# triq-org/spectroplot-js

Measured on AMD Instinct MI355X. Metric: STFT frames/sec (N=1024 cf32) + IQ MSamples/s end-to-end to RGBA, higher is better.
Workload: dtype f64; 1 GPU; 16 MSample cf32, N=1024, Blackman-Harris, Viridis, gain 6, range 30, spectrogram layout, 16384 frames per GPU; format=CF32, n=1024, samples_per_gpu=16777216, frames_per_gpu=16384, window=blackmanHarris, cmap=viridis, generator=trinoise seed=0x5EED0001 step=7321 gshift=11 amp=0.5 namp=0.02

## Files before the change

### include/spectroplot_hip.h

```cpp
#ifndef SPECTROPLOT_HIP_H
#define SPECTROPLOT_HIP_H

#include <stddef.h>
#include <stdint.h>

#ifdef __cplusplus
extern "C" {
#endif

#define SP_VERSION 100
#define SP_CB_HIST_SIZE 1000
#define SP_MAX_LUT 4096
#define SP_MAX_N (1 << 20)

enum sp_status {
    SP_OK = 0,
    SP_ERR_INVALID_ARG = -1,
    SP_ERR_NOT_POW2 = -2,
    SP_ERR_BYTE_LENGTH = -3,
    SP_ERR_UNSUPPORTED = -4,
    SP_ERR_NO_DEVICE = -5,
    SP_ERR_HIP = -6,
    SP_ERR_NOMEM = -7
};
// ... 73 lines not shown
    int32_t n;
    int32_t channel_mode, waterfall;
    double gain, range;
} sp_named_request;
int sp_render_named(sp_context *ctx, const sp_named_request *req, const uint8_t *bytes, size_t nbytes, int32_t width, const sp_reply *reply);
int sp_render_named_ex(sp_context *ctx, const sp_named_request *req, int32_t detector, const uint8_t *bytes, size_t nbytes, int32_t width,
                       const sp_reply *reply);
int sp_named_resolve(const char *window, const char *cmap, const char **window_name, const char **cmap_key, int32_t *lut_len);
int sp_context_plan_creations(const sp_context *ctx, int64_t *count);

int sp_plan_create(sp_context *ctx, const sp_request *req, sp_plan **plan);
void sp_plan_destroy(sp_plan *plan);
int sp_plan_execute(sp_plan *plan, const void *d_bytes, size_t nbytes, int32_t width, const sp_reply *d_reply);
int sp_plan_execute_from_host(sp_plan *plan, const uint8_t *bytes, size_t nbytes, int32_t width, const sp_reply *d_reply);
int sp_merge_replies(sp_context *ctx, const void *d_records, int32_t count, int32_t lut_len, uint64_t *d_c_hist, uint64_t *d_cb_hist,
                     double *d_dbfs_minmax);
int sp_merge_replies_batch(sp_context *ctx, const void *d_gathered, int32_t ranks, int32_t renders, int32_t lut_len, void *d_merged);
int sp_place_strips(sp_context *ctx, uint8_t *d_image, const uint8_t *d_strips, int32_t count, int32_t n, int32_t width,
                    int32_t slice_width, int32_t waterfall);
typedef struct sp_group sp_group;
enum sp_group_gather { SP_GROUP_GATHER_DEVICE = 0, SP_GROUP_GATHER_HOST = 1 };
int sp_group_create(const int32_t *devices, int32_t count, sp_group **group);
void sp_group_destroy(sp_group *group);
int sp_group_size(const sp_group *group);
int sp_group_render(sp_group *group, const sp_request *req, const uint8_t *bytes, size_t nbytes, int32_t width, const sp_reply *reply);
int sp_group_render_ex(sp_group *group, const sp_request *req, const uint8_t *bytes, size_t nbytes, int32_t width, const sp_reply *reply,
                       int32_t gather);
const char *sp_group_transport(const sp_group *group);
const char *sp_group_transport_note(const sp_group *group);
int sp_group_last_timings(const sp_group *group, double *render_ms, double *gather_ms, double *download_ms);
int sp_group_rccl_info(const sp_group *group, char *text, size_t capacity);
int sp_group_root_bytes(const sp_group *group, size_t *image_bytes, size_t *staging_bytes);
const char *sp_group_last_error(const sp_group *group);

typedef struct sp_batch_item {
    const void *bytes;
    size_t nbytes;
    int32_t width;
    int32_t reserved;
    sp_reply reply;
} sp_batch_item;
int sp_plan_execute_batch(sp_plan *plan, const sp_batch_item *items, int32_t count);
int sp_render_batch(sp_context *ctx, const sp_request *req, const sp_batch_item *items, int32_t count);
int sp_debug_batch_plan(int32_t format, int32_t n, int32_t lut_len, int32_t cu_count, const size_t *nbytes, const int32_t *widths,
                        int32_t count, int64_t *out, size_t capacity, size_t *used);

int sp_plan_debug_launch(const sp_plan *plan, size_t nbytes, int32_t width, const void *rgba, int64_t *out, size_t capacity, size_t *used);
int sp_debug_frames_launch(int32_t n, int32_t lut_len, int64_t count, int32_t cu_count, int32_t gf_fixed, int64_t *out, size_t capacity,
                           size_t *used);

const char *sp_plan_kernel_name(const sp_plan *plan);
const char *sp_plan_kernel_name_for(const sp_plan *plan, size_t nbytes, int32_t width);
int sp_plan_force_kernel(sp_plan *plan, int32_t which);

int sp_plan_execute_traces(sp_plan *plan, const void *d_bytes, size_t nbytes, int32_t width, double *d_trace_min, double *d_trace_max);
int sp_render_traces(sp_context *ctx, const sp_request *req, const uint8_t *bytes, size_t nbytes, int32_t width, double *trace_min,
                     double *trace_max);
const char *sp_plan_traces_kernel_name_for(const sp_plan *plan, size_t nbytes, int32_t width);

int sp_plan_execute_power(sp_plan *plan, const void *d_bytes, size_t nbytes, int32_t width, double *d_power);
int sp_plan_power_to_db(sp_plan *plan, const double *d_power, size_t count, double *d_db);
int sp_render_power(sp_context *ctx, const sp_request *req, const uint8_t *bytes, size_t nbytes, int32_t width, int32_t db, double *power);
const char *sp_plan_power_kernel_name_for(const sp_plan *plan, size_t nbytes, int32_t width);

int sp_power_mean(sp_context *ctx, const double *d_power, int32_t n, int32_t width, double *d_mean);
int sp_plan_execute_mean(sp_plan *plan, const void *d_bytes, size_t nbytes, int32_t width, double *d_mean);
int sp_render_mean(sp_context *ctx, const sp_request *req, const uint8_t *bytes, size_t nbytes, int32_t width, int32_t db, double *mean);
int sp_context_set_mean_window(sp_context *ctx, size_t bytes);
int sp_debug_exact_sum(const double *values, size_t count, double *sum);
const char *sp_plan_mean_kernel_name_for(const sp_plan *plan, size_t nbytes, int32_t width);

#define SP_MAX_BANDS 64
int sp_band_rows(int32_t n, double f_lo, double f_hi, int32_t *y0, int32_t *y1);
int sp_power_bands(sp_context *ctx, const double *d_power, int32_t n, int32_t width, const int32_t *bands, int32_t count, double *d_band);
int sp_plan_execute_bandpower(sp_plan *plan, const void *d_bytes, size_t nbytes, int32_t width, const int32_t *bands, int32_t count,
                              double *d_band);
int sp_render_bandpower(sp_context *ctx, const sp_request *req, const uint8_t *bytes, size_t nbytes, int32_t width, const int32_t *bands,
                        int32_t count, int32_t db, double *band);
const char *sp_plan_bandpower_kernel_name_for(const sp_plan *plan, size_t nbytes, int32_t width);

int sp_power_tracks(sp_context *ctx, const double *d_power, int32_t n, int32_t width, const int32_t *bands, int32_t count,
                    int32_t *d_row, double *d_peak);
int sp_plan_execute_track(sp_plan *plan, const void *d_bytes, size_t nbytes, int32_t width, const int32_t *bands, int32_t count,
                          int32_t *d_row, double *d_peak);
int sp_render_track(sp_context *ctx, const sp_request *req, const uint8_t *bytes, size_t nbytes, int32_t width, const int32_t *bands,
                    int32_t count, int32_t db, int32_t *row, double *peak);
const char *sp_plan_track_kernel_name_for(const sp_plan *plan, size_t nbytes, int32_t width);
int sp_debug_band_peak(const double *values, int32_t n, int32_t y0, int32_t y1, int32_t *row, double *peak);

#define SP_OCCUPANCY_TILE_ROWS 4096
int sp_power_occupancy(sp_context *ctx, const double *d_power, int32_t n, int32_t width, const double *d_threshold, const int32_t *bands,
                       int32_t count, uint32_t *d_rows, uint32_t *d_frames);
int sp_plan_execute_occupancy(sp_plan *plan, const void *d_bytes, size_t nbytes, int32_t width, const double *d_threshold,
                              const int32_t *bands, int32_t count, uint32_t *d_rows, uint32_t *d_frames);
int sp_render_occupancy(sp_context *ctx, const sp_request *req, const uint8_t *bytes, size_t nbytes, int32_t width, const double *threshold,
                        const int32_t *bands, int32_t count, uint32_t *rows, uint32_t *frames);
const char *sp_plan_occupancy_kernel_name_for(const sp_plan *plan, size_t nbytes, int32_t width);
int sp_debug_occupancy(const double *values, const double *thresholds, int32_t n, int32_t y0, int32_t y1, uint32_t *count);

int sp_plan_execute_index(sp_plan *plan, const void *d_bytes, size_t nbytes, int32_t width, const sp_reply *d_reply, uint8_t *d_index);
int sp_render_index(sp_context *ctx, const sp_request *req, const uint8_t *bytes, size_t nbytes, int32_t width, const sp_reply *reply,
                    uint8_t *index);
int sp_index_to_rgba(sp_context *ctx, const uint8_t *d_index, size_t pixels, const uint8_t *lut_rgb, int32_t lut_len, uint8_t *d_rgba);
const char *sp_plan_index_kernel_name_for(const sp_plan *plan, size_t nbytes, int32_t width);
int sp_plan_debug_index_launch(const sp_plan *plan, size_t nbytes, int32_t width, const void *index, int64_t *out, size_t capacity,
                               size_t *used);
// ... 31 lines not shown
```

### spectroplot-js_amd/binding.py

```python
import ctypes as C
import math
import os
import weakref
import subprocess

import numpy as np

_HERE = os.path.dirname(os.path.abspath(__file__))

SP_CB_HIST_SIZE = 1000
FORMATS = ["CU4", "CS4", "CU8", "CS8", "CU12", "CS12", "CU16", "CS16", "CU32", "CS32", "CU64", "CS64", "CF32", "CF64"]

SP_ERR_NOT_POW2 = -2
SP_ERR_BYTE_LENGTH = -3
SP_ERR_UNSUPPORTED = -4
SP_ERR_NO_DEVICE = -5
SP_ERR_INVALID_ARG = -1

DETECTORS = {"sample": 0, "peak": 1}


def detector_id(detector):
    if detector not in DETECTORS:
        raise SpectroplotError(SP_ERR_INVALID_ARG, "detector must be 'sample' or 'peak', not %r" % (detector,))
# ... 36 lines not shown
def build_library(force=False):
    target = lib_path()
    if force:
        subprocess.check_call(["make", "-s", "-C", _HERE, "clean"])
    subprocess.check_call(["make", "-s", "-C", _HERE])
    return target


class Library:
    _instance = None

    def __init__(self, path=None):
        path = path or lib_path()
        if not os.path.exists(path):
            raise SpectroplotError(SP_ERR_NO_DEVICE, "HIP library %s is missing: run __graft_entry__.build() first" % path)
        L = self.L = C.CDLL(path)
        self.path = path
        vp, i32, sz, dbl = C.c_void_p, C.c_int32, C.c_size_t, C.c_double
        L.sp_version.restype = C.c_int
        L.sp_status_string.restype = C.c_char_p
        L.sp_status_string.argtypes = [C.c_int]
        L.sp_last_error.restype = C.c_char_p
        L.sp_last_error.argtypes = [vp]
        L.sp_format_parse.argtypes = [C.c_char_p, C.POINTER(i32), C.POINTER(i32)]
        L.sp_format_element_size.argtypes = [i32]
        L.sp_slice_bounds.argtypes = [sz, i32, i32, i32, C.POINTER(sz), C.POINTER(sz)]
        L.sp_window.argtypes = [C.c_char_p, i32, vp, C.POINTER(dbl)]
        L.sp_twiddles.argtypes = [i32, vp, vp]
        L.sp_js_log10.restype = dbl
        L.sp_js_log10.argtypes = [dbl]
        L.sp_cmap_count.restype = C.c_int
        L.sp_cmap_key.restype = C.c_char_p
        L.sp_cmap_key.argtypes = [i32]
        L.sp_cmap.argtypes = [C.c_char_p, vp, i32, C.POINTER(i32)]
        L.sp_cmap_generate.argtypes = [C.c_char_p, i32, vp]
        L.sp_plan_execute_from_host.argtypes = [vp, vp, sz, i32, C.POINTER(_Reply)]
        L.sp_device_count.argtypes = [C.POINTER(i32)]
        L.sp_context_create.argtypes = [i32, C.POINTER(vp)]
        L.sp_context_destroy.argtypes = [vp]
        L.sp_context_destroy.restype = None
        L.sp_context_set_stream.argtypes = [vp, vp]
        L.sp_context_synchronize.argtypes = [vp]
        L.sp_render.argtypes = [vp, C.POINTER(_Request), vp, sz, i32, C.POINTER(_Reply)]
        L.sp_render_named.argtypes = [vp, C.POINTER(_NamedRequest), vp, sz, i32, C.POINTER(_Reply)]
        L.sp_named_resolve.argtypes = [C.c_char_p, C.c_char_p, C.POINTER(C.c_char_p), C.POINTER(C.c_char_p), C.POINTER(i32)]
        L.sp_context_plan_creations.argtypes = [vp, C.POINTER(C.c_int64)]
        L.sp_plan_create.argtypes = [vp, C.POINTER(_Request), C.POINTER(vp)]
        L.sp_plan_destroy.argtypes = [vp]
        L.sp_plan_destroy.restype = None
        L.sp_plan_execute.argtypes = [vp, vp, sz, i32, C.POINTER(_Reply)]
        L.sp_plan_kernel_name.restype = C.c_char_p
        L.sp_plan_kernel_name.argtypes = [vp]
        L.sp_plan_force_kernel.argtypes = [vp, i32]
        L.sp_device_alloc.argtypes = [vp, sz, C.POINTER(vp)]
        L.sp_device_free.argtypes = [vp, vp]
        L.sp_device_upload.argtypes = [vp, vp, vp, sz]
        L.sp_device_download.argtypes = [vp, vp, vp, sz]
        L.sp_device_memset.argtypes = [vp, vp, C.c_int, sz]
        L.sp_synth_trinoise.argtypes = [vp, vp, i32, C.c_uint64, C.c_uint64, C.c_uint32, C.c_uint32, C.c_uint32, dbl, dbl]
        L.sp_context_last_kernel_ms.argtypes = [vp, C.POINTER(C.c_float)]
        L.sp_context_enable_timing.argtypes = [vp, i32]
        L.sp_merge_replies.argtypes = [vp, vp, i32, i32, vp, vp, vp]
        L.sp_merge_replies_batch.argtypes = [vp, vp, i32, i32, i32, vp]
        L.sp_context_event_pair_overhead_ms.argtypes = [vp, C.POINTER(C.c_float)]
        L.sp_place_strips.argtypes = [vp, vp, vp, i32, i32, i32, i32, i32]
        if not hasattr(L, "sp_group_create"):
            return
        L.sp_group_create.argtypes = [C.POINTER(i32), i32, C.POINTER(vp)]
        L.sp_group_destroy.argtypes = [vp]
        L.sp_group_destroy.restype = None
        L.sp_group_size.argtypes = [vp]
        L.sp_group_render.argtypes = [vp, C.POINTER(_Request), vp, sz, i32, C.POINTER(_Reply)]
        L.sp_group_transport.restype = C.c_char_p
        L.sp_group_transport.argtypes = [vp]
        L.sp_group_last_error.restype = C.c_char_p
        L.sp_group_last_error.argtypes = [vp]
        if hasattr(L, "sp_group_render_ex"):
            L.sp_group_render_ex.argtypes = [vp, C.POINTER(_Request), vp, sz, i32, C.POINTER(_Reply), i32]
            L.sp_group_transport_note.restype = C.c_char_p
            L.sp_group_transport_note.argtypes = [vp]
            L.sp_group_last_timings.argtypes = [vp, C.POINTER(dbl), C.POINTER(dbl), C.POINTER(dbl)]
            L.sp_group_root_bytes.argtypes = [vp, C.POINTER(sz), C.POINTER(sz)]
            if hasattr(L, "sp_group_rccl_info"):
                L.sp_group_rccl_info.argtypes = [vp, C.c_char_p, sz]
            L.sp_render_strip.argtypes = [vp, C.POINTER(_Request), vp, sz, i32, C.POINTER(_Reply), i32]
        if hasattr(L, "sp_context_last_upload_bytes"):
            L.sp_context_last_upload_bytes.argtypes = [vp, C.POINTER(sz)]
        L.sp_context_get_stream.argtypes = [vp, C.POINTER(vp)]
        L.sp_plan_execute_batch.argtypes = [vp, C.POINTER(_BatchItem), i32]
        L.sp_render_batch.argtypes = [vp, C.POINTER(_Request), C.POINTER(_BatchItem), i32]
        L.sp_debug_batch_plan.argtypes = [i32, i32, i32, i32, vp, vp, i32, vp, sz, C.POINTER(sz)]
        L.sp_peak_subframes.argtypes = [i32, i32, sz, i32, C.POINTER(i32), C.POINTER(i32)]
        L.sp_render_named_ex.argtypes = [vp, C.POINTER(_NamedRequest), i32, vp, sz, i32, C.POINTER(_Reply)]
        L.sp_plan_kernel_name_for.restype = C.c_char_p
        L.sp_plan_kernel_name_for.argtypes = [vp, sz, i32]
        L.sp_plan_debug_launch.argtypes = [vp, sz, i32, vp, vp, sz, C.POINTER(sz)]
        L.sp_debug_frames_launch.argtypes = [i32, i32, C.c_int64, i32, i32, vp, sz, C.POINTER(sz)]
        L.sp_plan_execute_traces.argtypes = [vp, vp, sz, i32, vp, vp]
        L.sp_render_traces.argtypes = [vp, C.POINTER(_Request), vp, sz, i32, vp, vp]
        L.sp_plan_traces_kernel_name_for.restype = C.c_char_p
        L.sp_plan_traces_kernel_name_for.argtypes = [vp, sz, i32]
        L.sp_plan_execute_power.argtypes = [vp, vp, sz, i32, vp]
        L.sp_plan_power_to_db.argtypes = [vp, vp, sz, vp]
        L.sp_render_power.argtypes = [vp, C.POINTER(_Request), vp, sz, i32, i32, vp]
        L.sp_plan_power_kernel_name_for.restype = C.c_char_p
        L.sp_plan_power_kernel_name_for.argtypes = [vp, sz, i32]
# ... 483 lines not shown
    def density_from_index(self, d_index, n, width, waterfall, lut_len, d_density, accumulate=False):
        self._chk(self.lib.L.sp_density_from_index(self.h, C.c_void_p(d_index or None), int(n), int(width), int(bool(waterfall)),
                                                   int(lut_len), C.c_void_p(d_density or None), int(bool(accumulate))))

    def plan_creations(self):
        n = C.c_int64()
        self._chk(self.lib.L.sp_context_plan_creations(self.h, C.byref(n)))
        return n.value

    def plan(self, fmt, n, windowc, block_norm, gain, rng, lut, channel_mode=False, waterfall=False, detector="sample"):
        return Plan(self, fmt, n, windowc, block_norm, gain, rng, lut, channel_mode, waterfall, detector)


class Plan:

    def __init__(self, ctx, fmt, n, windowc, block_norm, gain, rng, lut, channel_mode=False, waterfall=False, detector="sample"):
        self.ctx = ctx
        self.detector = detector
        self.n = int(n)
        self.fid, self.sample_width = parse_format(fmt)
        req, keep = _make_request(self.fid, n, windowc, block_norm, gain, rng, lut, channel_mode, waterfall, detector)
        self.lut_len = len(keep[1])
        h = C.c_void_p()
        ctx._chk(ctx.lib.L.sp_plan_create(ctx.h, C.byref(req), C.byref(h)))
        self.h = h
        ctx._plans.add(self)

    def close(self):
        if self.h:
            self.ctx.lib.L.sp_plan_destroy(self.h)
            self.h = None

    def __del__(self):
        try:
            self.close()
        except Exception:
            pass

    def kernel_name(self, nbytes=None, width=None):
        if nbytes is None:
            return self.ctx.lib.L.sp_plan_kernel_name(self.h).decode()
        return self.ctx.lib.L.sp_plan_kernel_name_for(self.h, int(nbytes), int(width)).decode()

    def debug_launch(self, nbytes, width, rgba=0):
        out = np.zeros(len(LAUNCH_FIELDS), np.int64)
        used = C.c_size_t()
        self.ctx._chk(self.ctx.lib.L.sp_plan_debug_launch(self.h, int(nbytes), int(width), C.c_void_p(rgba or None),
                                                          out.ctypes.data_as(C.c_void_p), len(out), C.byref(used)))
        return _launch_dict(out)

    def force_kernel(self, which):
        self.ctx._chk(self.ctx.lib.L.sp_plan_force_kernel(self.h, {"auto": 0, "scratch": 1, "frames": 3}[which]))

    def execute(self, d_bytes, nbytes, width, rgba=0, gauge_mins=0, gauge_maxs=0, gauge_amps=0, c_hist=0, cb_hist=0, dbfs_minmax=0):
        rep = _device_reply(rgba, gauge_mins, gauge_maxs, gauge_amps, c_hist, cb_hist, dbfs_minmax)
        self.ctx._chk(self.ctx.lib.L.sp_plan_execute(self.h, C.c_void_p(d_bytes), nbytes, int(width), C.byref(rep)))

    def _kernel_name_for(self, kind, nbytes, width):
        return getattr(self.ctx.lib.L, "sp_plan_%s_kernel_name_for" % kind)(self.h, int(nbytes), int(width)).decode()

    def traces_kernel_name_for(self, nbytes, width):
        return self._kernel_name_for("traces", nbytes, width)

    def execute_traces(self, d_bytes, nbytes, width, trace_min=0, trace_max=0):
        self.ctx._chk(self.ctx.lib.L.sp_plan_execute_traces(self.h, C.c_void_p(d_bytes or None), int(nbytes), int(width),
                                                            C.c_void_p(trace_min or None), C.c_void_p(trace_max or None)))

    def power_kernel_name_for(self, nbytes, width):
        return self._kernel_name_for("power", nbytes, width)

    def execute_power(self, d_bytes, nbytes, width, d_power):
        self.ctx._chk(self.ctx.lib.L.sp_plan_execute_power(self.h, C.c_void_p(d_bytes or None), int(nbytes), int(width),
                                                           C.c_void_p(d_power or None)))

    def mean_kernel_name_for(self, nbytes, width):
        return self._kernel_name_for("mean", nbytes, width)

    def execute_mean(self, d_bytes, nbytes, width, d_mean):
        self.ctx._chk(self.ctx.lib.L.sp_plan_execute_mean(self.h, C.c_void_p(d_bytes or None), int(nbytes), int(width),
                                                          C.c_void_p(d_mean or None)))

    def bandpower_kernel_name_for(self, nbytes, width):
        return self._kernel_name_for("bandpower", nbytes, width)

    def execute_bandpower(self, d_bytes, nbytes, width, bands, d_band):
        b, count = _band_array(bands)
        self.ctx._chk(self.ctx.lib.L.sp_plan_execute_bandpower(self.h, C.c_void_p(d_bytes or None), int(nbytes), int(width),
                                                               _p(b) if count else None, count, C.c_void_p(d_band or None)))

    def track_kernel_name_for(self, nbytes, width):
        return self._kernel_name_for("track", nbytes, width)

    def execute_track(self, d_bytes, nbytes, width, bands, d_row, d_peak):
        b, count = _band_array(bands)
        self.ctx._chk(self.ctx.lib.L.sp_plan_execute_track(self.h, C.c_void_p(d_bytes or None), int(nbytes), int(width),
                                                           _p(b) if count else None, count, C.c_void_p(d_row or None),
                                                           C.c_void_p(d_peak or None)))

    def occupancy_kernel_name_for(self, nbytes, width):
        return self._kernel_name_for("occupancy", nbytes, width)

    def execute_occupancy(self, d_bytes, nbytes, width, d_threshold, bands, d_rows, d_frames):
        b, count = _band_array(bands)
        self.ctx._chk(self.ctx.lib.L.sp_plan_execute_occupancy(self.h, C.c_void_p(d_bytes or None), int(nbytes), int(width),
                                                               C.c_void_p(d_threshold or None), _p(b) if count else None, count,
                                                               C.c_void_p(d_rows or None), C.c_void_p(d_frames or None)))
# ... 102 lines not shown
```

### spectroplot-js_amd/csrc/sp_api.hip

```cpp
#include <hip/hip_runtime.h>

#include <cmath>
#include <cstdio>
#include <cstdlib>
#include <cstring>
#include <new>
#include <string>
#include <vector>

#include "../../include/spectroplot_hip.h"
#include "sp_geometry.h"
#include "sp_host.h"
#include "sp_kernel_frames_batch.h"
#include "sp_kernel_frames_peak.h"
#include "sp_kernel_frames_traces.h"
#include "sp_kernel_frames_power.h"
#include "sp_kernel_frames_index.h"
#include "sp_launch.h"
#include "sp_exact_sum.h"
#include "sp_track_core.h"
#include "sp_occupancy_core.h"
#include "sp_cmap_tables.h"

namespace {

struct DeviceBuffer {
    void *p = nullptr;
    size_t cap = 0;
    int reserve(size_t bytes)
    {
        if (bytes <= cap) return SP_OK;
        if (p) (void)hipFree(p);
        p = nullptr;
        cap = 0;
        size_t want = bytes + bytes / 8 + 256;
        if (hipMalloc(&p, want) != hipSuccess) {
            if (hipMalloc(&p, bytes) != hipSuccess) return SP_ERR_NOMEM;
            want = bytes;
        }
        cap = want;
        return SP_OK;
    }
    void release()
    {
        if (p) (void)hipFree(p);
        p = nullptr;
        cap = 0;
    }
};

struct HostBuffer {
    void *p = nullptr;
    size_t cap = 0;
    int reserve(size_t bytes)
    {
        if (bytes <= cap) return SP_OK;
        if (p) (void)hipHostFree(p);
        p = nullptr;
        cap = 0;
        const size_t want = bytes + bytes / 8 + 256;
        if (hipHostMalloc(&p, want, hipHostMallocDefault) != hipSuccess) return SP_ERR_NOMEM;
        cap = want;
        return SP_OK;
    }
    void release()
    {
        if (p) (void)hipHostFree(p);
        p = nullptr;
        cap = 0;
    }
};

struct NamedRequest {
    std::string format, window, cmap;
    int32_t n = 0, channel_mode = 0, waterfall = 0;
    double gain = 0, range = 0;
    std::vector<double> windowc;
    std::vector<uint8_t> lut;
    double block_norm = 0;
    static std::string str(const char *s) { return s ? s : ""; }
    bool same(const sp_named_request &r) const
    {
        return !windowc.empty() && format == str(r.format) && window == str(r.window) && cmap == str(r.cmap) && n == r.n
               && channel_mode == (r.channel_mode ? 1 : 0) && waterfall == (r.waterfall ? 1 : 0) && !memcmp(&gain, &r.gain, 8)
               && !memcmp(&range, &r.range, 8);
    }
};

}

struct sp_context {
    int device = 0;
    hipStream_t own_stream = nullptr;
    hipStream_t stream = nullptr;
    std::string error;
    int cu_count = 256;
    DeviceBuffer frame_minmax;
    DeviceBuffer partial;
    DeviceBuffer scratch;
    DeviceBuffer traces_ws;
    DeviceBuffer power_plane;
    DeviceBuffer mean_ws;
    DeviceBuffer plane_window;
    size_t mean_window_bytes = 0;
    DeviceBuffer index_rgba;
    DeviceBuffer density_index;
    DeviceBuffer density_reply;
    DeviceBuffer in_bytes, out_rgba, render_small;
    HostBuffer host_small;
    hipStream_t copy_in = nullptr, copy_out = nullptr;
    hipEvent_t ev_arrived[spgeo::kMaxChunks] = {}, ev_rendered[spgeo::kMaxChunks] = {};
    sp_plan *cached_plan = nullptr;
    NamedRequest named;
    long long plans_created = 0;
    bool acc_dirty = false;
    size_t last_upload_bytes = 0;
    int last_chunks = 0;
    uint32_t seq = 0;
    DeviceBuffer batch_dev;
    HostBuffer batch_host;
    hipEvent_t ev_batch = nullptr;
    hipEvent_t ev_batch_done = nullptr;
    bool timing = false;
    hipEvent_t ev0 = nullptr, ev1 = nullptr;
    bool timed = false;
};

enum Kernel {
    kKernelAuto = 0,
    kKernelScratch = 1,
    kKernelLdsR16 = 2,
    kKernelFrames = 3,
    kKernelFramesPeak = 4,
};
static bool finishes_request(int kernel) { return kernel == kKernelFrames || kernel == kKernelFramesPeak; }

struct sp_plan {
    sp_context *ctx = nullptr;
    sp_request req{};
    std::vector<double> window;
    std::vector<uint8_t> lut;
    int levels = 0;
    spfmt::Format fmt{};
    double block_norm_db = 0;
    float gray_a = 0, gray_b = 0, cb_a = 0, cb_b = 0;
    bool edges_in_f32 = false;
    bool taper_finite = false;
    bool tw16_ok = false;
    sphost::Thresholds th{};
    DeviceBuffer tables;
    const double *d_window = nullptr, *d_cos = nullptr, *d_sin = nullptr, *d_gray_edge = nullptr, *d_cb_edge = nullptr;
    const uint32_t *d_lut = nullptr;
    const uint16_t *d_cell_g = nullptr, *d_cell_l = nullptr;
    const double2 *d_stage_tw = nullptr;
    DeviceBuffer ident_lut;
    int force_kernel = kKernelAuto;
};

namespace {

int fail(sp_context *ctx, int code, const std::string &msg)
{
    if (ctx) ctx->error = msg;
    return code;
}

int hip_fail(sp_context *ctx, hipError_t e, const char *what)
{
    return fail(ctx, SP_ERR_HIP, std::string(what) + ": " + hipGetErrorString(e));
}

#define SP_HIP(ctx, call)                                            \
    do {                                                             \
        hipError_t e_ = (call);                                      \
        if (e_ != hipSuccess) return hip_fail((ctx), e_, #call);     \
    } while (0)

int validate_request(sp_context *ctx, const sp_request *r)
{
    std::string why;
    const int rc = sphost::validate_request(r, why);
    return rc ? fail(ctx, rc, why) : SP_OK;
}

template <typename Body>
int timed(sp_context *ctx, Body &&body)
{
    if (ctx->timing) SP_HIP(ctx, hipEventRecord(ctx->ev0, ctx->stream));
    const int rc = body();
    if (rc) return rc;
    if (ctx->timing) {
        SP_HIP(ctx, hipEventRecord(ctx->ev1, ctx->stream));
        ctx->timed = true;
    }
    return SP_OK;
}

}


extern "C" int sp_version(void) { return SP_VERSION; }

extern "C" const char *sp_status_string(int status)
{
    switch (status) {
    case SP_OK: return "ok";
    case SP_ERR_INVALID_ARG: return "invalid argument";
    case SP_ERR_NOT_POW2: return "Length is not a power of 2";
    case SP_ERR_BYTE_LENGTH: return "byte length is not a multiple of the element size";
// ... 399 lines not shown
extern "C" int sp_context_plan_creations(const sp_context *ctx, int64_t *count)
{
    if (!ctx || !count) return SP_ERR_INVALID_ARG;
    *count = (int64_t)ctx->plans_created;
    return SP_OK;
}

extern "C" void sp_plan_destroy(sp_plan *plan)
{
    if (!plan) return;
    if (plan->ctx) {
        (void)hipSetDevice(plan->ctx->device);
        (void)hipStreamSynchronize(plan->ctx->stream);
        if (plan->ctx->cached_plan == plan) plan->ctx->cached_plan = nullptr;
    }
    plan->tables.release();
    plan->ident_lut.release();
    delete plan;
}

static bool plan_frames_capable(const sp_plan *plan)
{
    return spk2::frames_kernel_supports(plan->req.n) && plan->req.lut_len >= 2 && plan->req.lut_len <= spk::kLdsMaxLut
           && plan->gray_b <= spk::kLdsMaxGrayB && plan->edges_in_f32 && plan->taper_finite && plan->th.frames_ok && plan->tw16_ok;
}

static int plan_kernel(const sp_plan *plan)
{
    if (plan->force_kernel) return plan->force_kernel;
#ifdef SP_EXPERIMENT_KNOBS
    static const int env_kernel = getenv("SP_FORCE_KERNEL") ? atoi(getenv("SP_FORCE_KERNEL")) : 0;
    if (env_kernel == kKernelFrames && plan_frames_capable(plan)) return kKernelFrames;
    if (env_kernel == kKernelScratch) return kKernelScratch;
#endif
    return plan_frames_capable(plan) ? kKernelFrames : kKernelScratch;
}

static int request_kernel(const sp_plan *plan, int32_t peak_m)
{
    const int k = plan_kernel(plan);
    if (plan->req.detector != SP_DETECTOR_PEAK || peak_m < 2) return k;
    return k == kKernelFrames && spk2::frames_peak_supports(plan->req.n) ? kKernelFramesPeak : kKernelScratch;
}

extern "C" int sp_plan_force_kernel(sp_plan *plan, int32_t which)
{
    if (!plan || which < kKernelAuto || which > kKernelFrames) return SP_ERR_INVALID_ARG;
    if (which == kKernelLdsR16) return fail(plan->ctx, SP_ERR_UNSUPPORTED, "k_lds_r16 is no longer part of the library");
    if (which == kKernelFrames && !plan_frames_capable(plan)) return fail(plan->ctx, SP_ERR_UNSUPPORTED, "k_frames does not cover this request");
    plan->force_kernel = which;
    return SP_OK;
}

static const char *kernel_name(int kernel)
{
    return kernel == kKernelFramesPeak ? "frames_peak" : kernel == kKernelFrames ? "frames" : "scratch_radix2";
}

extern "C" const char *sp_plan_kernel_name(const sp_plan *plan) { return plan ? kernel_name(request_kernel(plan, 2)) : ""; }

extern "C" const char *sp_plan_kernel_name_for(const sp_plan *plan, size_t nbytes, int32_t width)
{
    return plan ? kernel_name(request_kernel(plan, spgeo::peak_shape(spgeo::geometry(plan->fmt, plan->req.n, nbytes, width)).m)) : "";
}

struct PackedSource {
    const void *bytes;
    size_t nbytes;
    double stride;
};

static void plan_frame_args(const sp_plan *plan, spk::FrameArgs &a)
{
    a.n = plan->req.n;
    a.levels = plan->levels;
    a.channel_mode = plan->req.channel_mode ? 1 : 0;
    a.waterfall = plan->req.waterfall ? 1 : 0;
    a.lut_len = plan->req.lut_len;
    a.sample_width = plan->fmt.width;
    a.window = plan->d_window;
    a.cos_t = plan->d_cos;
    a.sin_t = plan->d_sin;
    a.gray_edge = plan->d_gray_edge;
    a.cb_edge = plan->d_cb_edge;
    a.lut_rgba = plan->d_lut;
    a.gray_a = plan->gray_a;
    a.gray_b = plan->gray_b;
    a.cb_a = plan->cb_a;
    a.cb_b = plan->cb_b;
    a.g2_a = plan->th.g2_a;
    a.g2_b = plan->th.g2_b;
    a.g2_thr = plan->th.g2_thr;
    a.g2_m = plan->th.g2_m;
    a.c2_a = plan->th.c2_a;
    a.c2_b = plan->th.c2_b;
    a.c2_thr = plan->th.c2_thr;
    a.c2_m = plan->th.c2_m;
    a.c2_lo = plan->th.c2_lo;
    a.c2_hi = plan->th.c2_hi;
    a.block_norm_db = plan->block_norm_db;
    a.gain = plan->req.gain;
    a.range = plan->req.range;
    a.cell_g = plan->d_cell_g;
    a.cell_l = plan->d_cell_l;
    a.cells = plan->th.cells;
}
// ... 140 lines not shown
        }
        return SP_OK;
    }

    const int which = request_kernel(plan, peak.m);
    if (src && which != kKernelFrames) return fail(ctx, SP_ERR_INVALID_ARG, "a packed source is for the frame-loop kernel only");
    rc = finishes_request(which) ? SP_OK : ctx->frame_minmax.reserve(2 * (size_t)width * sizeof(double));
    if (rc) return fail(ctx, rc, "workspace: out of device memory");
    const size_t acc_bytes = 64 + (SP_MAX_LUT + SP_CB_HIST_SIZE) * sizeof(unsigned long long);
    const bool fresh_partial = ctx->partial.cap < acc_bytes;
    rc = ctx->partial.reserve(acc_bytes);
    if (rc) return fail(ctx, rc, "workspace: out of device memory");
    if (first && (fresh_partial || ctx->acc_dirty)) {
        static const unsigned long long mm_init[2] = {0x7ff0000000000000ull, 0ull};
        SP_HIP(ctx, hipMemsetAsync(ctx->partial.p, 0, ctx->partial.cap, s));
        SP_HIP(ctx, hipMemcpyAsync((char *)ctx->partial.p + 16, mm_init, sizeof mm_init, hipMemcpyHostToDevice, s));
        SP_HIP(ctx, hipStreamSynchronize(s));
    }
    ctx->acc_dirty = true;

    spk::FrameArgs a{};
    plan_frame_args(plan, a);
    frame_source_args(a, plan, d_bytes, g, x_begin, x_end, src);
    a.frame_min = (double *)ctx->frame_minmax.p;
    a.frame_max = a.frame_min + width;
    a.scratch = nullptr;
    if (first && ++ctx->seq == 0) ctx->seq = 1;
    a.first = first ? 1 : 0;
    a.seq = ctx->seq;
    a.flag = (unsigned int *)ctx->partial.p;
    a.gauge_mins = out->gauge_mins;
    a.gauge_maxs = out->gauge_maxs;
    a.gauge_amps = out->gauge_amps;
    a.out_c = (unsigned long long *)out->c_hist;
    a.out_cb = (unsigned long long *)out->cb_hist;
    a.out_minmax = out->dbfs_minmax;

    a.mm_acc = (unsigned long long *)((char *)ctx->partial.p + 16);
    a.c_hist = (unsigned long long *)((char *)ctx->partial.p + 64);
    a.cb_hist = a.c_hist + SP_MAX_LUT;
    const bool extract = pic.kind == Picture::kIndexExtract;
    a.rgba = extract ? (uint8_t *)ctx->index_rgba.p : pic.image;
    a.rgba_fast = pic.kind == Picture::kIndexFrames ? index_fast(a.rgba, width, n, x_begin, x_end) : rgba_fast(a.rgba, width, n);
    if (extract) a.lut_rgba = (const uint32_t *)plan->ident_lut.p;

    const int32_t peak_nsamp = (int32_t)(peak.nsamp < 2147483647 ? peak.nsamp : 2147483647);
    rc = timed(ctx, [&]() -> int {
        int r = SP_OK;
        if (pic.kind == Picture::kIndexFrames) {
            if (which != kKernelFrames) return fail(ctx, SP_ERR_INVALID_ARG, "k_frames_index renders what k_frames renders");
            r = spk2::launch_frames_index(a, plan->req.format, plan->d_stage_tw, ctx->cu_count, ctx->device, s);
            if (r) return fail(ctx, r, "k_frames_index launch rejected the configuration");
        } else if (which == kKernelFrames) {
            r = spk2::launch_frames(a, plan->req.format, plan->d_stage_tw, ctx->cu_count, ctx->device, s);
            if (r) return fail(ctx, r, "k_frames launch rejected the configuration");
        } else if (which == kKernelFramesPeak) {
            r = spk2::launch_frames_peak(a, plan->req.format, plan->d_stage_tw, peak.m, peak_nsamp, ctx->cu_count, ctx->device, s);
            if (r) return fail(ctx, r, "k_frames_peak launch rejected the configuration");
        } else {
            const bool hold = peak.m >= 2;
            unsigned blocks;
            r = scratch_reserve(ctx, a, hold ? 3 : 2, x_end - x_begin, &blocks);
            if (r) return r;
            r = spk::launch_scratch_radix2(a, plan->req.format, blocks, hold, peak.m, peak_nsamp, s);
            if (r) return fail(ctx, r, "bad format");
        }
        SP_HIP(ctx, hipGetLastError());
        if (extract && x_end > x_begin) return extract_index_band(ctx, a.rgba, pic.image, width, n, plan->req.waterfall != 0, x_begin, x_end);
        return SP_OK;
    });
    if (rc) return rc;

    if (!last) return SP_OK;
    if (finishes_request(which)) {
        ctx->acc_dirty = false;
        return SP_OK;
    }

    spk::FinishArgs fa{};
    fa.bytes = a.bytes;
    fa.nbytes = a.nbytes;
    fa.nelem = a.nelem;
    fa.stride = a.stride;
    fa.n = n;
    fa.width = width;
    fa.format = plan->req.format;
    fa.block_norm_db = plan->block_norm_db;
    fa.gain = plan->req.gain;
    fa.range = plan->req.range;
    fa.frame_min = a.frame_min;
    fa.frame_max = a.frame_max;
    fa.gauge_mins = out->gauge_mins;
    fa.gauge_maxs = out->gauge_maxs;
    fa.gauge_amps = out->gauge_amps;
    fa.mm_acc = a.mm_acc;
    fa.out_minmax = out->dbfs_minmax;
    fa.lut_len = plan->req.lut_len;
    fa.acc_c = a.c_hist;
    fa.acc_cb = a.cb_hist;
    fa.out_c = (unsigned long long *)out->c_hist;
    fa.out_cb = (unsigned long long *)out->cb_hist;
    spk::launch_finish_frames(fa, s);
    SP_HIP(ctx, hipGetLastError());
    ctx->acc_dirty = false;
    return SP_OK;
}

extern "C" int sp_plan_execute(sp_plan *plan, const void *d_bytes, size_t nbytes, int32_t width, const sp_reply *out)
{
    if (!plan || !out) return SP_ERR_INVALID_ARG;
    return plan_execute_range(plan, d_bytes, request_shape(plan, nbytes, width), 0, width < 0 ? 0 : width, true, true, out,
                              Picture{Picture::kRgba, out->rgba});
}

extern "C" int sp_plan_debug_launch(const sp_plan *plan, size_t nbytes, int32_t width, const void *rgba, int64_t *out, size_t capacity,
                                    size_t *used)
{
    if (!plan || !plan->ctx || width < 0 || !used) return SP_ERR_INVALID_ARG;
    const RequestShape shape = request_shape(plan, nbytes, width);
    const spgeo::Geometry &g = shape.g;
    const int n = plan->req.n, cu_count = plan->ctx->cu_count;
    const int which = width == 0 ? kKernelAuto : request_kernel(plan, shape.peak.m);
    spk2::FramesLaunch fl{0, 0, 0, 0};
    int prefetch = 0;
    if (finishes_request(which)) {
        prefetch = spk2::frames_prefetch_width(plan->fmt.width, g.in_bounds, g.stride, g.width);
        if (spk2::frames_launch_rule(n, plan->req.lut_len, width, cu_count, 0, fl)) return SP_ERR_UNSUPPORTED;
    }
    const int64_t v[] = {which, plan->levels, plan->req.channel_mode ? 1 : 0, prefetch, fl.gf, fl.groups, fl.grid, fl.lds_bytes,
                         rgba_fast((const uint8_t *)rgba, width, n) ? 1 : 0, shape.peak.m, cu_count};
    *used = sizeof v / sizeof v[0];
    if (*used > capacity || !out) return SP_ERR_INVALID_ARG;
    memcpy(out, v, sizeof v);
    return SP_OK;
}

extern "C" int sp_debug_frames_launch(int32_t n, int32_t lut_len, int64_t count, int32_t cu_count, int32_t gf_fixed, int64_t *out,
                                      size_t capacity, size_t *used)
{
    if (n < 2 || sphost::log2_exact(n) < 0 || count < 1 || count > 2147483647 || cu_count < 1 || gf_fixed < 0 || !used) return SP_ERR_INVALID_ARG;
    spk2::FramesLaunch fl{0, 0, 0, 0};
    const int rc = spk2::frames_launch_rule(n, lut_len, count, cu_count, gf_fixed, fl);
    if (rc) return rc;
    const int64_t v[] = {fl.gf, fl.groups, fl.grid, fl.lds_bytes};
    *used = sizeof v / sizeof v[0];
    if (*used > capacity || !out) return SP_ERR_INVALID_ARG;
    memcpy(out, v, sizeof v);
    return SP_OK;
}


extern "C" int sp_merge_replies(sp_context *ctx, const void *d_records, int32_t count, int32_t lut_len, uint64_t *d_c_hist,
                                uint64_t *d_cb_hist, double *d_dbfs_minmax)
{
    if (!ctx || !d_records || count < 1 || lut_len < 1 || lut_len > SP_MAX_LUT) return SP_ERR_INVALID_ARG;
    SP_HIP(ctx, hipSetDevice(ctx->device));
    spk::launch_merge_replies((const unsigned long long *)d_records, count, lut_len, sphost::ReplyRecord{(size_t)lut_len, 0}.words(), 1,
                              (unsigned long long *)d_c_hist, (unsigned long long *)d_cb_hist, d_dbfs_minmax, ctx->stream);
    SP_HIP(ctx, hipGetLastError());
    return SP_OK;
}

extern "C" int sp_merge_replies_batch(sp_context *ctx, const void *d_gathered, int32_t ranks, int32_t renders, int32_t lut_len, void *d_merged)
{
    if (!ctx || !d_gathered || !d_merged || ranks < 1 || renders < 1 || renders > 65535 || lut_len < 1 || lut_len > SP_MAX_LUT)
        return SP_ERR_INVALID_ARG;
    SP_HIP(ctx, hipSetDevice(ctx->device));
    const sphost::ReplyRecord rec{(size_t)lut_len, 0};
    const sp_reply m = rec.view(d_merged);
    spk::launch_merge_replies((const unsigned long long *)d_gathered, ranks, lut_len, (size_t)renders * rec.words(), renders,
                              (unsigned long long *)m.c_hist, (unsigned long long *)m.cb_hist, m.dbfs_minmax, ctx->stream);
    SP_HIP(ctx, hipGetLastError());
    return SP_OK;
}


extern "C" int sp_place_strips(sp_context *ctx, uint8_t *d_image, const uint8_t *d_strips, int32_t count, int32_t n, int32_t width,
                               int32_t slice_width, int32_t waterfall)
{
    if (!ctx || !d_image || !d_strips || count < 1 || n < 1 || width < 1 || slice_width < 0) return SP_ERR_INVALID_ARG;
    if ((int64_t)count * slice_width > width) return fail(ctx, SP_ERR_INVALID_ARG, "strips do not fit the image");
    if (slice_width == 0) return SP_OK;
    SP_HIP(ctx, hipSetDevice(ctx->device));
    const bool wide = (slice_width & 3) == 0 && (width & 3) == 0 && (((uintptr_t)d_image | (uintptr_t)d_strips) & 15) == 0
                      && (!waterfall || (n & 3) == 0);
    const int rc = spk::launch_place_strips(wide, d_image, d_strips, count, n, width, slice_width, waterfall, ctx->stream);
    if (rc) return fail(ctx, rc, "image too large for one placement launch");
// ... 1510 lines not shown
```

Measured before the change: 254.0 million frames/s.

## Add warp-specialized split-set frames kernel overlapping FFT with RGBA drain

Adds a sibling k_frames_sets kernel for N=1024 spectrogram RGBA output. It splits each workgroup's waves into two sets that alternate tile halves and coordinate through LDS counters, so draining the pixel rows of the previous group overlaps with the FFT of the next. The kernel is enabled by default and chosen whenever its narrow conditions hold; otherwise the existing frames kernel runs. It adds a larger LDS layout, spin-wait synchronisation with a trap on timeout, and a new routing path that could deadlock or lose occupancy if the assumptions are off.

Result: no change. 253.6 million frames/s (-0.2%).

```diff
diff --git a/include/spectroplot_hip.h b/include/spectroplot_hip.h
--- a/include/spectroplot_hip.h
+++ b/include/spectroplot_hip.h
@@ -149,6 +149,11 @@
 const char *sp_plan_kernel_name(const sp_plan *plan);
 const char *sp_plan_kernel_name_for(const sp_plan *plan, size_t nbytes, int32_t width);
 int sp_plan_force_kernel(sp_plan *plan, int32_t which);
+int sp_plan_set_frames_sets(sp_plan *plan, int on);
+int sp_plan_debug_frames_sets(const sp_plan *plan, size_t nbytes, int32_t width, const void *rgba);
+int sp_plan_last_frames_sets(const sp_plan *plan);
+int sp_debug_frames_sets_applies(int32_t n, int32_t lut_len, int32_t prefetch, int32_t channel_mode, int32_t waterfall, int32_t has_rgba,
+                                 int32_t rgba_fast, int64_t frames, int32_t cu_count);
 
 int sp_plan_execute_traces(sp_plan *plan, const void *d_bytes, size_t nbytes, int32_t width, double *d_trace_min, double *d_trace_max);
 int sp_render_traces(sp_context *ctx, const sp_request *req, const uint8_t *bytes, size_t nbytes, int32_t width, double *trace_min,
diff --git a/spectroplot-js_amd/binding.py b/spectroplot-js_amd/binding.py
--- a/spectroplot-js_amd/binding.py
+++ b/spectroplot-js_amd/binding.py
@@ -112,6 +112,10 @@
         L.sp_plan_kernel_name.restype = C.c_char_p
         L.sp_plan_kernel_name.argtypes = [vp]
         L.sp_plan_force_kernel.argtypes = [vp, i32]
+        L.sp_plan_set_frames_sets.argtypes = [vp, C.c_int]
+        L.sp_plan_debug_frames_sets.argtypes = [vp, sz, i32, vp]
+        L.sp_plan_last_frames_sets.argtypes = [vp]
+        L.sp_debug_frames_sets_applies.argtypes = [i32, i32, i32, i32, i32, i32, i32, C.c_int64, i32]
         L.sp_device_alloc.argtypes = [vp, sz, C.POINTER(vp)]
         L.sp_device_free.argtypes = [vp, vp]
         L.sp_device_upload.argtypes = [vp, vp, vp, sz]
@@ -701,6 +705,21 @@
     def force_kernel(self, which):
         self.ctx._chk(self.ctx.lib.L.sp_plan_force_kernel(self.h, {"auto": 0, "scratch": 1, "frames": 3}[which]))
 
+    def set_frames_sets(self, on):
+        self.ctx._chk(self.ctx.lib.L.sp_plan_set_frames_sets(self.h, 1 if on else 0))
+
+    def debug_frames_sets(self, nbytes, width, rgba=0):
+        r = self.ctx.lib.L.sp_plan_debug_frames_sets(self.h, int(nbytes), int(width), C.c_void_p(rgba or None))
+        if r < 0:
+            self.ctx._chk(r)
+        return bool(r)
+
+    def last_frames_sets(self):
+        r = self.ctx.lib.L.sp_plan_last_frames_sets(self.h)
+        if r < 0:
+            self.ctx._chk(r)
+        return bool(r)
+
     def execute(self, d_bytes, nbytes, width, rgba=0, gauge_mins=0, gauge_maxs=0, gauge_amps=0, c_hist=0, cb_hist=0, dbfs_minmax=0):
         rep = _device_reply(rgba, gauge_mins, gauge_maxs, gauge_amps, c_hist, cb_hist, dbfs_minmax)
         self.ctx._chk(self.ctx.lib.L.sp_plan_execute(self.h, C.c_void_p(d_bytes), nbytes, int(width), C.byref(rep)))
diff --git a/spectroplot-js_amd/csrc/sp_api.hip b/spectroplot-js_amd/csrc/sp_api.hip
--- a/spectroplot-js_amd/csrc/sp_api.hip
+++ b/spectroplot-js_amd/csrc/sp_api.hip
@@ -16,6 +16,7 @@
 #include "sp_kernel_frames_traces.h"
 #include "sp_kernel_frames_power.h"
 #include "sp_kernel_frames_index.h"
+#include "sp_kernel_frames_sets.h"
 #include "sp_launch.h"
 #include "sp_exact_sum.h"
 #include "sp_track_core.h"
@@ -95,6 +96,7 @@
     hipStream_t stream = nullptr;
     std::string error;
     int cu_count = 256;
+    bool last_frames_sets = false;
     DeviceBuffer frame_minmax;
     DeviceBuffer partial;
     DeviceBuffer scratch;
@@ -155,6 +157,7 @@
     const double2 *d_stage_tw = nullptr;
     DeviceBuffer ident_lut;
     int force_kernel = kKernelAuto;
+    bool frames_sets = true;
 };
 
 namespace {
@@ -660,6 +663,38 @@
     return SP_OK;
 }
 
+extern "C" int sp_plan_set_frames_sets(sp_plan *plan, int on)
+{
+    if (!plan) return SP_ERR_INVALID_ARG;
+    plan->frames_sets = on != 0;
+    return SP_OK;
+}
+
+extern "C" int sp_plan_last_frames_sets(const sp_plan *plan)
+{
+    if (!plan || !plan->ctx) return SP_ERR_INVALID_ARG;
+    return plan->ctx->last_frames_sets ? 1 : 0;
+}
+
+extern "C" int sp_debug_frames_sets_applies(int32_t n, int32_t lut_len, int32_t prefetch, int32_t channel_mode, int32_t waterfall,
+                                            int32_t has_rgba, int32_t rgba_fast, int64_t frames, int32_t cu_count)
+{
+    if (frames < 1 || frames > 2147483647 || cu_count < 1) return SP_ERR_INVALID_ARG;
+    spk2::FramesLaunch fl{0, 0, 0, 0};
+    const int rc = spk2::frames_launch_rule(n, lut_len, frames, cu_count, 0, fl);
+    if (rc) return rc;
+    spk::FrameArgs a{};
+    a.n = n;
+    a.lut_len = lut_len;
+    a.channel_mode = channel_mode;
+    a.waterfall = waterfall;
+    a.rgba = has_rgba ? (uint8_t *)16 : nullptr;
+    a.rgba_fast = rgba_fast;
+    a.frame0 = 0;
+    a.x_end = (int)frames;
+    return spk2::frames_sets_applies(a, prefetch, fl, spk2::layout_sets(n, lut_len, fl.gf).total) ? 1 : 0;
+}
+
 static const char *kernel_name(int kernel)
 {
     return kernel == kKernelFramesPeak ? "frames_peak" : kernel == kKernelFrames ? "frames" : "scratch_radix2";
@@ -906,7 +941,7 @@
             r = spk2::launch_frames_index(a, plan->req.format, plan->d_stage_tw, ctx->cu_count, ctx->device, s);
             if (r) return fail(ctx, r, "k_frames_index launch rejected the configuration");
         } else if (which == kKernelFrames) {
-            r = spk2::launch_frames(a, plan->req.format, plan->d_stage_tw, ctx->cu_count, ctx->device, s);
+            r = spk2::launch_frames_routed(a, plan->req.format, plan->d_stage_tw, ctx->cu_count, ctx->device, s, plan->frames_sets, &ctx->last_frames_sets);
             if (r) return fail(ctx, r, "k_frames launch rejected the configuration");
         } else if (which == kKernelFramesPeak) {
             r = spk2::launch_frames_peak(a, plan->req.format, plan->d_stage_tw, peak.m, peak_nsamp, ctx->cu_count, ctx->device, s);
@@ -987,6 +1022,24 @@
     if (*used > capacity || !out) return SP_ERR_INVALID_ARG;
     memcpy(out, v, sizeof v);
     return SP_OK;
+}
+
+extern "C" int sp_plan_debug_frames_sets(const sp_plan *plan, size_t nbytes, int32_t width, const void *rgba)
+{
+    if (!plan || !plan->ctx || width < 0) return SP_ERR_INVALID_ARG;
+    if (width == 0 || !plan->frames_sets) return 0;
+    const RequestShape shape = request_shape(plan, nbytes, width);
+    if (request_kernel(plan, shape.peak.m) != kKernelFrames) return 0;
+    spk::FrameArgs a{};
+    plan_frame_args(plan, a);
+    a.rgba = (uint8_t *)rgba;
+    a.rgba_fast = rgba_fast(a.rgba, width, plan->req.n);
+    a.frame0 = 0;
+    a.x_end = width;
+    spk2::FramesLaunch fl{0, 0, 0, 0};
+    if (spk2::frames_launch_rule(a.n, a.lut_len, width, plan->ctx->cu_count, 0, fl)) return SP_ERR_UNSUPPORTED;
+    const int prefetch = spk2::frames_prefetch_width(plan->fmt.width, shape.g.in_bounds, shape.g.stride, shape.g.width);
+    return spk2::frames_sets_applies(a, prefetch, fl, spk2::layout_sets(a.n, a.lut_len, fl.gf).total) ? 1 : 0;
 }
 
 extern "C" int sp_debug_frames_launch(int32_t n, int32_t lut_len, int64_t count, int32_t cu_count, int32_t gf_fixed, int64_t *out,
diff --git a/spectroplot-js_amd/csrc/sp_frames_sets_body.inc.h b/spectroplot-js_amd/csrc/sp_frames_sets_body.inc.h
--- /dev/null
+++ b/spectroplot-js_amd/csrc/sp_frames_sets_body.inc.h
@@ -0,0 +1,94 @@
+#define layout layout_sets
+#include "sp_frames_setup.inc.h"
+#undef layout
+
+#include "sp_frames_raw_regs.inc.h"
+#include "sp_frames_request.inc.h"
+    const bool owner = blockIdx.x == 0 && __builtin_amdgcn_readfirstlane(tid >> 6) == 0 && a.first;
+#include "sp_frames_prologue_consts.inc.h"
+    {
+#include "sp_frames_table_loads.inc.h"
+#include "sp_frames_reply_clear.inc.h"
+        request(a.frame0 + (xcd * chunk + lane_in_xcd) * group_frames + fs0);
+#include "sp_frames_table_stores.inc.h"
+    }
+#include "sp_frames_taper.inc.h"
+
+    const spfmt::View view{a.bytes, a.nbytes, a.nelem};
+    uint32_t pf_word = 0;
+#include "sp_frames_epilogue_consts.inc.h"
+
+#include "sp_frames_writeout.inc.h"
+    const int wave = __builtin_amdgcn_readfirstlane(tid >> 6);
+    const bool set_a = wave < 4;
+    const unsigned done_addr = (unsigned)__builtin_amdgcn_readfirstlane((int)(unsigned)(size_t)(const __attribute__((address_space(3))) unsigned int *)s_done);
+    const SetCounter a_meet{done_addr + 8}, a_wrote{done_addr + 12}, b_meet{done_addr + 16}, b_done{done_addr + 20};
+    unsigned a_meets = 0;
+    unsigned char *const s_tile_all = s_tile;
+    const double *const edge_cb_global = a.cb_edge;
+    (void)edge_cb;
+    (void)drain;
+    const int half_rows = group_frames / 2;
+    auto drain_b_quarter = [&](const int bx0, const int k, const int part, const int nparts) {
+        const int row0 = half_rows + (k & 1) * half_rows;
+        drain_rows(bx0 + half_rows - row0, wave + 4 * part, 4 * nparts, row0, half_rows, wave * 64, 64, true);
+    };
+#ifdef SP_STAMPS
+    [[maybe_unused]] unsigned long long stamp_slow = 0;
+#endif
+    int kk = 0;
+    int b_next = 0;
+    int prev_x0 = -1;
+    int b_slice_x0 = -1;
+    int drain_x0 = -1;
+    int gpar = 0;
+    meet.arrive();
+    for (int g = xcd * chunk + lane_in_xcd; g < g_end; g += per_xcd) {
+        const int x0 = a.frame0 + g * group_frames;
+        if (kk >= 2) {
+            if (set_a) {
+                if (b_next < kk - 1) {
+                    b_done.wait_for(4u * (unsigned)(kk - 1));
+                    drain_b_quarter(prev_x0 - per_xcd * group_frames, kk - 2, 0, 1);
+                    side_outputs(prev_x0 - per_xcd * group_frames, gpar);
+                    a_wrote.arrive();
+                    b_next = kk - 1;
+                }
+                a_meet.arrive();
+                a_meet.wait_for(4u * ++a_meets);
+            } else {
+                a_wrote.wait_for(4u * (unsigned)(kk - 1));
+            }
+        }
+        unsigned char *const s_tile_set = s_tile_all + (set_a ? 0 : (kk & 1) * half_rows * tile_pitch);
+        for (int r = 0; r < rounds; r++) {
+#define SP_X_END a.x_end
+#include "sp_frames_slot_deal.inc.h"
+#undef SP_X_END
+            const int64_t start = frame_start(a.stride, x);
+            double2 *const centre = tl == 0 ? &s_amp[gpar * group_frames + fr] : nullptr;
+#include "sp_frames_frame_regs.inc.h"
+#define SP_TOUCH_AHEAD
+#include "sp_frames_next_frame.inc.h"
+#undef SP_TOUCH_AHEAD
+
+#include "sp_frames_sets_passes.inc.h"
+            {
+                unsigned char *const s_tile = s_tile_set;
+                const double *const edge_cb = edge_cb_global;
+#include "sp_frames_pixels.inc.h"
+            }
+#include "sp_frames_publish.inc.h"
+        }
+        if (!set_a) {
+            b_meet.arrive();
+            b_meet.wait_for(4u * (unsigned)(kk + 1));
+            b_done.arrive();
+        }
+        drain_x0 = x0;
+        prev_x0 = x0;
+        gpar ^= 1;
+        kk++;
+    }
+
+#include "sp_frames_sets_finale.inc.h"
diff --git a/spectroplot-js_amd/csrc/sp_frames_sets_finale.inc.h b/spectroplot-js_amd/csrc/sp_frames_sets_finale.inc.h
--- /dev/null
+++ b/spectroplot-js_amd/csrc/sp_frames_sets_finale.inc.h
@@ -0,0 +1,46 @@
+    const LateArgs la = late_args();
+#define SP_LUT_LEN a.lut_len
+#define SP_CELLS a.cells
+#define SP_REPLY la
+#define SP_AFTER_CELLS_READ
+#include "sp_frames_hist_ranges.inc.h"
+    const unsigned int seen = __hip_atomic_load(la->flag, __ATOMIC_RELAXED, __HIP_MEMORY_SCOPE_AGENT);
+    if (set_a && b_next < kk - 1) {
+        b_done.wait_for(4u * (unsigned)(kk - 1));
+        drain_b_quarter(prev_x0 - per_xcd * group_frames, kk - 2, 0, 1);
+        side_outputs(prev_x0 - per_xcd * group_frames, gpar);
+    }
+    if (drain_x0 >= 0) {
+        const int half = tid >> 8;
+        const SetCounter last_meet{done_addr + 4u * (unsigned)__builtin_amdgcn_readfirstlane(half)};
+        last_meet.arrive();
+        last_meet.wait_for(4u);
+        const int row0 = half * (half_rows + ((kk - 1) & 1) * half_rows);
+        drain_rows(drain_x0 + half * half_rows - row0, 0, 1, row0, half_rows, half * (kThreads / 2), kThreads / 2, true);
+    }
+    lds_barrier();
+    {
+        constexpr int kPer = 3;
+        static_assert(kThreads * kPer >= kMaxCells, "every cell needs a thread");
+        unsigned int *const s_pre = (unsigned int *)(smem + kOffXch);
+        unsigned int *const s_part = s_pre + kThreads * kPer + 4;
+#include "sp_frames_hist_scan.inc.h"
+        if (seen != la->seq) {
+            unsigned polls = 0;
+            while (__hip_atomic_load(la->flag, __ATOMIC_RELAXED, __HIP_MEMORY_SCOPE_AGENT) != la->seq) {
+                __builtin_amdgcn_s_sleep(32);
+                if (++polls > (1u << 22)) __builtin_trap();
+            }
+        }
+#include "sp_frames_hist_adds.inc.h"
+        if (drain_x0 >= 0) side_outputs(drain_x0, gpar ^ 1);
+        lds_barrier();
+        double *const out_mm = la->out_minmax;
+        if (tid < 2 && out_mm) {
+#include "sp_frames_range_atomics.inc.h"
+        }
+    }
+#undef SP_LUT_LEN
+#undef SP_CELLS
+#undef SP_REPLY
+#undef SP_AFTER_CELLS_READ
diff --git a/spectroplot-js_amd/csrc/sp_frames_sets_passes.inc.h b/spectroplot-js_amd/csrc/sp_frames_sets_passes.inc.h
--- /dev/null
+++ b/spectroplot-js_amd/csrc/sp_frames_sets_passes.inc.h
@@ -0,0 +1,29 @@
+            unsigned tw_off = 0;
+            asm volatile("" : "+s"(tw_off));
+            const double2 *tw = stage_tw + tw_off;
+            if (set_a) {
+                if (drain_x0 >= 0) {
+                    a_meet.arrive();
+                    a_meet.wait_for(4u * ++a_meets);
+                    drain_rows(drain_x0, 0, 2, 0, half_rows, 0, kThreads / 2, true);
+                } else if (b_next < kk && b_done.peek() >= 4u * (unsigned)(b_next + 1)) {
+                    b_slice_x0 = prev_x0;
+                    drain_b_quarter(b_slice_x0, b_next, 0, 2);
+                }
+            }
+#include "sp_frames_fft.inc.h"
+
+            if (set_a) {
+                if (drain_x0 >= 0) {
+                    drain_rows(drain_x0, 1, 2, 0, half_rows, 0, kThreads / 2, true);
+                    a_meet.arrive();
+                    a_meet.wait_for(4u * ++a_meets);
+                    drain_x0 = -1;
+                } else if (b_slice_x0 >= 0) {
+                    drain_b_quarter(b_slice_x0, b_next, 1, 2);
+                    side_outputs(b_slice_x0, gpar ^ 1);
+                    a_wrote.arrive();
+                    b_next++;
+                    b_slice_x0 = -1;
+                }
+            }
diff --git a/spectroplot-js_amd/csrc/sp_inst_frames_sets.hip b/spectroplot-js_amd/csrc/sp_inst_frames_sets.hip
--- /dev/null
+++ b/spectroplot-js_amd/csrc/sp_inst_frames_sets.hip
@@ -0,0 +1,2 @@
+#define SP_INST_SETS
+#include "sp_kernel_frames_sets.h"
diff --git a/spectroplot-js_amd/csrc/sp_kernel_frames_sets.h b/spectroplot-js_amd/csrc/sp_kernel_frames_sets.h
--- /dev/null
+++ b/spectroplot-js_amd/csrc/sp_kernel_frames_sets.h
@@ -0,0 +1,143 @@
+#pragma once
+
+#include "sp_kernel_frames.h"
+
+namespace spk2 {
+
+constexpr int kSetsLog2N = 10;
+constexpr int kSetsPrefetch = 8;
+
+__host__ __device__ inline Layout layout_sets(int n, int lut_len, int group_frames)
+{
+    Layout l;
+    const int fpb = kFrameThreads * 16 / n;
+    int o = kOffXch + fpb * (n + n / 16) * 8;
+    l.off_tw = o;     o += frames_tw_entries(n) * 16;
+    l.off_gedge = o;  o += lut_len * 8;
+    o = (o + 15) & ~15;
+    l.off_mm = o;     o += 2 * group_frames * mm_slots(n) * 2 * 8;
+    l.off_tile = o;   o += ((group_frames + group_frames / 2) * (n + kTilePad) + 15) & ~15;
+    l.off_cbedge = l.off_tile;
+    l.off_done = o;   o += 32;
+    o = (o + 15) & ~15;
+    l.off_amp = o;    o += 16 + 2 * group_frames * 16;
+    l.off_win = o;    o += n * 8;
+    l.total = (o + 15) & ~15;
+    return l;
+}
+
+struct SetCounter {
+    unsigned addr;
+    __device__ inline void arrive() const
+    {
+        unsigned long long save;
+        unsigned a_v, one_v;
+        asm volatile("v_mov_b32 %[a_v], %[addr]\n\t"
+                     "v_mov_b32 %[one_v], 1\n\t"
+                     "s_mov_b64 %[save], exec\n\t"
+                     "s_mov_b64 exec, 1\n\t"
+                     "ds_add_u32 %[a_v], %[one_v]\n\t"
+                     "s_mov_b64 exec, %[save]"
+                     : [save] "=&s"(save), [a_v] "=&v"(a_v), [one_v] "=&v"(one_v)
+                     : [addr] "s"(addr)
+                     : "memory");
+    }
+    __device__ inline unsigned peek() const
+    {
+        unsigned a_v, got_v, got_s;
+        asm volatile("v_mov_b32 %[a_v], %[addr]\n\t"
+                     "ds_read_b32 %[got_v], %[a_v]\n\t"
+                     "s_waitcnt lgkmcnt(0)\n\t"
+                     "v_readfirstlane_b32 %[got_s], %[got_v]"
+                     : [a_v] "=&v"(a_v), [got_v] "=&v"(got_v), [got_s] "=&s"(got_s)
+                     : [addr] "s"(addr)
+                     : "memory");
+        return got_s;
+    }
+    __device__ inline void wait_for(unsigned target_any) const
+    {
+        const unsigned target = (unsigned)__builtin_amdgcn_readfirstlane((int)target_any);
+        unsigned a_v, got_v, got_s, polls;
+        asm volatile("v_mov_b32 %[a_v], %[addr]\n\t"
+                     "s_mov_b32 %[polls], 0\n"
+                     "L_sp_set_poll_%=:\n\t"
+                     "ds_read_b32 %[got_v], %[a_v]\n\t"
+                     "s_waitcnt lgkmcnt(0)\n\t"
+                     "v_readfirstlane_b32 %[got_s], %[got_v]\n\t"
+                     "s_sub_i32 %[got_s], %[got_s], %[target]\n\t"
+                     "s_cmp_ge_i32 %[got_s], 0\n\t"
+                     "s_cbranch_scc1 L_sp_set_done_%=\n\t"
+                     "s_sleep 2\n\t"
+                     "s_add_u32 %[polls], %[polls], 1\n\t"
+                     "s_cmp_lt_u32 %[polls], 0x400000\n\t"
+                     "s_cbranch_scc1 L_sp_set_poll_%=\n\t"
+                     "s_trap 2\n"
+                     "L_sp_set_done_%=:"
+                     : [a_v] "=&v"(a_v), [got_v] "=&v"(got_v), [got_s] "=&s"(got_s), [polls] "=&s"(polls)
+                     : [addr] "s"(addr), [target] "s"(target)
+                     : "memory", "scc");
+    }
+};
+
+template <int LOG2N, bool CH, int PFB>
+__global__ __launch_bounds__(kFrameThreads, 1) void k_frames_sets(const FrameArgs a, const int format, const double2 *__restrict__ stage_tw,
+                                                            const int group_frames, const int groups)
+{
+    static_assert(LOG2N == kSetsLog2N && !CH && PFB == kSetsPrefetch, "the sibling is built for one variant");
+#pragma push_macro("SP_STAMP")
+#pragma push_macro("SP_TAIL_STAMP")
+#undef SP_STAMP
+#undef SP_TAIL_STAMP
+#define SP_STAMP(k)
+#define SP_TAIL_STAMP(k)
+#include "sp_frames_sets_body.inc.h"
+#pragma pop_macro("SP_TAIL_STAMP")
+#pragma pop_macro("SP_STAMP")
+}
+
+inline int frames_min_groups_per_workgroup(int groups, int grid)
+{
+    const int per_xcd = grid >> 3, chunk = (groups + 7) >> 3;
+    int least = groups;
+    for (int xcd = 0; xcd < 8; xcd++) {
+        const int g_end = groups < (xcd + 1) * chunk ? groups : (xcd + 1) * chunk;
+        const int first = xcd * chunk + per_xcd - 1;
+        const int have = g_end > first ? (g_end - first + per_xcd - 1) / per_xcd : 0;
+        if (have < least) least = have;
+    }
+    return least;
+}
+
+inline bool frames_sets_applies(const FrameArgs &a, int prefetch, const FramesLaunch &fl, int lds_bytes)
+{
+    return a.n == (1 << kSetsLog2N) && prefetch == kSetsPrefetch && !a.channel_mode && !a.waterfall && a.rgba && a.rgba_fast && fl.gf == 32 &&
+           (a.x_end - a.frame0) % 32 == 0 && frames_min_groups_per_workgroup(fl.groups, fl.grid) >= 2 && lds_bytes <= 160 * 1024;
+}
+
+int launch_frames_sets_10(const FrameArgs &a, int format, const double2 *stage_tw, const FramesLaunch &fl, int lds_bytes, int device,
+                          hipStream_t stream);
+
+#ifdef SP_INST_SETS
+int launch_frames_sets_10(const FrameArgs &a, int format, const double2 *stage_tw, const FramesLaunch &fl, int lds_bytes, int device,
+                          hipStream_t stream)
+{
+    return launch_full_lds<k_frames_sets<kSetsLog2N, false, kSetsPrefetch>>(fl.grid, lds_bytes, device, stream, a, format, stage_tw, fl.gf,
+                                                                           fl.groups);
+}
+#endif
+
+inline int launch_frames_routed(const FrameArgs &a, int format, const double2 *stage_tw, int cu_count, int device, hipStream_t stream,
+                                bool sets_on, bool *took_sets)
+{
+    *took_sets = false;
+    if (sets_on && a.n == (1 << kSetsLog2N) && !a.channel_mode && !a.waterfall && a.rgba && a.rgba_fast) {
+        const int prefetch = frames_prefetch_width(a.sample_width, a.in_bounds, a.stride, a.width);
+        FramesLaunch fl;
+        if (frames_launch_rule(a.n, a.lut_len, a.x_end - a.frame0, cu_count, 0, fl)) return SP_ERR_UNSUPPORTED;
+        const int lds_bytes = layout_sets(a.n, a.lut_len, fl.gf).total;
+        if (frames_sets_applies(a, prefetch, fl, lds_bytes)) return *took_sets = true, launch_frames_sets_10(a, format, stage_tw, fl, lds_bytes, device, stream);
+    }
+    return launch_frames(a, format, stage_tw, cu_count, device, stream);
+}
+
+}
```
